# tensorlayer/HyperPose

Hardware: AMD Instinct MI355X
Metric: end-to-end FPS (preproc+DNN+PAF parse) @ 368x432 (higher is better)
Workload: dtype f32; 1 GPU; configs[1]: Lightweight-OpenPose (MobilenetDilated) + PAF parser, batch 8 @ 368x432 per GPU; frames from pinned host memory (one H2D per batch), parser on the network's own maps, humans to the host; key=configs[1]/f32, global_batch=8, parallelism=frame-sharded x1, no steady-state collective, pipes_per_gpu=4, parser_input=the network's own heat-maps

## Files before the change

hyperpose_amd/csrc/conv32_epilogue.hpp:

```cpp
#pragma once
#include "conv_fp32.hpp"

#include "conv_device.hpp"

namespace hp {

typedef float f32x4e __attribute__((ext_vector_type(4)));

template <int TM>
struct rows_geom {
    static constexpr int CH = TM * 32, PITCH = CH + 4, LPR = CH / 4, RPP = 64 / LPR, NP = 32 / RPP;
    static constexpr int SLAB_BYTES = 32 * PITCH * 4;
};

template <int TM, int NROWS, class F>
__device__ __forceinline__ void conv32_drain_rows(const conv32_params& p, const float* slab, int lane, int m_base, F&& pixel)
{
    using R = rows_geom<TM>;
    const int c4 = lane % R::LPR, r0 = lane / R::LPR;
    const int m = m_base + c4 * 4;
    const bool any = m < p.Cout, full = m + 3 < p.Cout;
    const bool out_vec = ((p.out.coff | p.out.cs) & 3) == 0, res_vec = p.res.p && ((p.res.coff | p.res.cs) & 3) == 0;
    const f32x4e bs = *reinterpret_cast<const f32x4e*>(p.bias + m);
    f32x4e sl = { p.act_slope, p.act_slope, p.act_slope, p.act_slope };
    if (p.alpha)
        sl = *reinterpret_cast<const f32x4e*>(p.alpha + m);
    constexpr int NPASS = NROWS / R::RPP, GRP = NPASS < 4 ? NPASS : NPASS % 4 == 0 ? 4 : NPASS % 3 == 0 ? 3 : 1;
    static_assert(NROWS % R::RPP == 0 && NPASS % GRP == 0, "slab rows per pass");
#pragma unroll
    for (int g = 0; g < NPASS; g += GRP) {
        f32x4e v[GRP], rr[GRP];
        bool ok[GRP];
        long ooff[GRP];
#pragma unroll
        for (int k = 0; k < GRP; ++k) {
            const int r = (g + k) * R::RPP + r0;
            long roff = 0;
            pixel(r, ok[k], ooff[k], roff);
            ok[k] = ok[k] && any;
            v[k] = *reinterpret_cast<const f32x4e*>(slab + r * R::PITCH + c4 * 4);
            rr[k] = f32x4e{ 0.f, 0.f, 0.f, 0.f };
            if (p.res.p && ok[k]) {
                if (full && res_vec)
                    rr[k] = *reinterpret_cast<const f32x4e*>(p.res.p + roff + m);
                else {
#pragma unroll
                    for (int e = 0; e < 4; ++e)
                        if (m + e < p.Cout)
                            rr[k][e] = p.res.p[roff + m + e];
                }
            }
        }
#pragma unroll
        for (int k = 0; k < GRP; ++k) {
            f32x4e o;
#pragma unroll
            for (int e = 0; e < 4; ++e) {
                float x = v[k][e] + bs[e];
                if (p.res.p && p.res_before_act)
                    x += rr[k][e];
                x = x > 0.f ? fminf(x, p.act_hi) : x * sl[e];
                if (p.res.p && !p.res_before_act)
                    x += rr[k][e];
                o[e] = x;
            }
            if (ok[k]) {
                if (full && out_vec)
                    *reinterpret_cast<f32x4e*>(p.out.p + ooff[k] + m) = o;
                else {
#pragma unroll
                    for (int e = 0; e < 4; ++e)
                        if (m + e < p.Cout)
                            p.out.p[ooff[k] + m + e] = o[e];
                }
            }
        }
    }
}

template <int TM, class F>
__device__ __forceinline__ void conv32_store_rows(const conv32_params& p, const floatx16 (&acc)[TM], float* slab, int lane, int m_base, F&& pixel)
{
    using R = rows_geom<TM>;
    const int n = lane & 31, fk = lane >> 5;
#pragma unroll
    for (int i = 0; i < TM; ++i)
#pragma unroll
        for (int q = 0; q < 4; ++q)
            *reinterpret_cast<f32x4e*>(slab + n * R::PITCH + 32 * i + 8 * q + 4 * fk) = f32x4e{ acc[i][4 * q], acc[i][4 * q + 1], acc[i][4 * q + 2], acc[i][4 * q + 3] };
    asm volatile("s_waitcnt lgkmcnt(0)" ::: "memory");
    conv32_drain_rows<TM, 32>(p, slab, lane, m_base, pixel);
}

}
```

hyperpose_amd/csrc/conv_fp32.hip:

```cpp
#include "conv_fp32.hpp"

#include "conv32_epilogue.hpp"
#include "conv_device.hpp"

#include <algorithm>
#include <cstdlib>

namespace hp {

namespace {

typedef float f32x4 __attribute__((ext_vector_type(4)));

__device__ __forceinline__ float act32(float v, int act, float param, float alpha)
{
    switch (act) {
    case ACT_RELU:
        return fmaxf(v, 0.f);
    case ACT_RELU6:
        return fminf(fmaxf(v, 0.f), 6.f);
    case ACT_LEAKY:
        return v > 0.f ? v : v * param;
    case ACT_PRELU:
        return v > 0.f ? v : v * alpha;
    case ACT_SIGMOID:
        return 1.f / (1.f + expf(-v));
    case ACT_SOFTPLUS:
        return v > 20.f ? v : log1pf(expf(v));
    default:
        return v;
    }
}

__device__ __forceinline__ long tv32_off(const tview32& t, int b, int y, int x)
{
    return ((long)b * t.img + (long)y * t.wp + x) * t.cs + t.coff;
}

}

template <int BM, int BN, int WM, int WN, bool ROWS>
__global__ __launch_bounds__(256) void conv32_kernel(const conv32_params p)
{
    constexpr int BK = 16, LDR = 20;
    constexpr int TM = BM / WM / 32, TN = BN / WN / 32, NA = BM / 64, NB = BN / 64;
    static_assert(WM * WN == 4 && TM >= 1 && TN >= 1 && NA >= 1 && NB >= 1, "tile");
    constexpr int AB_BYTES = 2 * (BM + BN) * LDR * 4, SLABS = 4 * rows_geom<TM>::SLAB_BYTES;
    __shared__ __attribute__((aligned(16))) unsigned char lds_raw[AB_BYTES > SLABS ? AB_BYTES : SLABS];
    float (*const sA)[BM * LDR] = reinterpret_cast<float (*)[BM * LDR]>(lds_raw);
    float (*const sB)[BN * LDR] = reinterpret_cast<float (*)[BN * LDR]>(lds_raw + 2 * BM * LDR * 4);

    const int tid = threadIdx.x, lane = tid & 63, wave = tid >> 6;
    const int wm = wave / WN, wn = wave % WN;
    const int G = p.Cout_pad / BM, nx = (p.npix + BN - 1) / BN;
    const int bj = blockIdx.x >> 3, ptile = (bj / G) * 8 + (blockIdx.x & 7);
    if (ptile >= nx)
        return;
    const int n0 = ptile * BN, m0 = (bj % G) * BM;
    const int lrow = tid >> 2, lchunk = (tid & 3) * 4;
    const int OHW = p.OH * p.OW, kc = p.Cin / BK, steps = p.KH * p.KW * kc;

    long bbase[NB];
#pragma unroll
    for (int j = 0; j < NB; ++j) {
        const int n = min(n0 + lrow + 64 * j, p.npix - 1);
        const int b = n / OHW, rem = n - b * OHW;
        const int oy = rem / p.OW, ox = rem - oy * p.OW;
        bbase[j] = tv32_off(p.in, b, oy * p.stride - p.pad_t, ox * p.stride - p.pad_l) + lchunk;
    }
    const float* const wrow = p.w + (long)(m0 + lrow) * p.Cin + lchunk;

    f32x4 ra[NA], rb[NB];
    auto gload = [&](int s) {
        const int tap = s / kc, k0 = (s - tap * kc) * BK;
        const int ky = tap / p.KW, kx = tap - ky * p.KW;
        const long toff = ((long)(ky * p.dil) * p.in.wp + kx * p.dil) * p.in.cs + k0;
        const float* const wt = wrow + (long)tap * p.Cout_pad * p.Cin + k0;
#pragma unroll
        for (int j = 0; j < NA; ++j)
            ra[j] = *reinterpret_cast<const f32x4*>(wt + (long)(64 * j) * p.Cin);
#pragma unroll
        for (int j = 0; j < NB; ++j)
            rb[j] = *reinterpret_cast<const f32x4*>(p.in.p + bbase[j] + toff);
    };
    auto to_lds = [&](int buf) {
#pragma unroll
        for (int j = 0; j < NA; ++j)
            *reinterpret_cast<f32x4*>(&sA[buf][(lrow + 64 * j) * LDR + lchunk]) = ra[j];
#pragma unroll
        for (int j = 0; j < NB; ++j)
            *reinterpret_cast<f32x4*>(&sB[buf][(lrow + 64 * j) * LDR + lchunk]) = rb[j];
    };

    floatx16 acc[TM][TN];
#pragma unroll
    for (int i = 0; i < TM; ++i)
#pragma unroll
        for (int j = 0; j < TN; ++j)
#pragma unroll
            for (int r = 0; r < 16; ++r)
                acc[i][j][r] = 0.f;

    const int frow = lane & 31, fh = (lane >> 5) * 4;
    int dbg_i = 0;
#define HP_STAMP()                                       \
    if (p.dbg && blockIdx.x == 9 && tid == 0)            \
        p.dbg[dbg_i++] = __builtin_amdgcn_s_memtime();
    HP_STAMP();
    if (p.dbg && tid == 0 && blockIdx.x < 4096) {
        p.dbg[128 + 3 * blockIdx.x] = __builtin_amdgcn_s_memrealtime();
        p.dbg[128 + 3 * blockIdx.x + 2] = ((unsigned long long)__builtin_amdgcn_s_getreg((31 << 11) | 20) << 32) | (unsigned)__builtin_amdgcn_s_getreg((31 << 11) | 4);
    }
    gload(0);
    to_lds(0);
    lds_barrier();
    HP_STAMP();
#pragma unroll 1
    for (int s = 0; s < steps; ++s) {
        gload(min(s + 1, steps - 1));
        const float* const a_s = &sA[s & 1][(wm * TM * 32 + frow) * LDR + fh];
        const float* const b_s = &sB[s & 1][(wn * TN * 32 + frow) * LDR + fh];
#pragma unroll
        for (int kk = 0; kk < BK / 8; ++kk) {
            f32x4 fa[TM], fb[TN];
#pragma unroll
            for (int i = 0; i < TM; ++i)
                fa[i] = *reinterpret_cast<const f32x4*>(a_s + i * 32 * LDR + kk * 8);
#pragma unroll
            for (int j = 0; j < TN; ++j)
                fb[j] = *reinterpret_cast<const f32x4*>(b_s + j * 32 * LDR + kk * 8);
#pragma unroll
            for (int e = 0; e < 4; ++e)
#pragma unroll
                for (int i = 0; i < TM; ++i)
#pragma unroll
                    for (int j = 0; j < TN; ++j)
                        acc[i][j] = __builtin_amdgcn_mfma_f32_32x32x2f32(fa[i][e], fb[j][e], acc[i][j], 0, 0, 0);
        }
        to_lds((s + 1) & 1);
        lds_barrier();
        if ((s & 7) == 7)
            HP_STAMP();
    }

    if constexpr (ROWS) {
        lds_barrier();
        float* const slab = reinterpret_cast<float*>(lds_raw) + wave * (rows_geom<TM>::SLAB_BYTES / 4);
#pragma unroll
        for (int j = 0; j < TN; ++j) {
            floatx16 fin[TM];
#pragma unroll
            for (int i = 0; i < TM; ++i)
                fin[i] = acc[i][j];
            const int nb = n0 + (wn * TN + j) * 32;
            conv32_store_rows<TM>(p, fin, slab, lane, m0 + wm * TM * 32, [&](int r, bool& ok, long& ooff, long& roff) {
                const int n = nb + r;
                ok = n < p.npix;
                const int nc = min(n, p.npix - 1);
                const int b = nc / OHW, rem = nc - b * OHW;
                const int oy = rem / p.OW, ox = rem - oy * p.OW;
                ooff = tv32_off(p.out, b, oy, ox);
                roff = p.res.p ? tv32_off(p.res, b, oy, ox) : 0;
            });
        }
    } else {
    const bool out_vec = p.out.p && ((p.out.coff | p.out.cs) & 3) == 0;
    const bool res_vec = p.res.p && ((p.res.coff | p.res.cs) & 3) == 0;
    const bool res_pre = p.res.p && p.res_before_act, res_post = p.res.p && !p.res_before_act;
#pragma unroll
    for (int j = 0; j < TN; ++j) {
        const int n = n0 + (wn * TN + j) * 32 + frow;
        const bool pix_ok = n < p.npix;
        const int nc = min(n, p.npix - 1);
        const int b = nc / OHW, rem = nc - b * OHW;
        const int oy = rem / p.OW, ox = rem - oy * p.OW;
        const long ooff = p.out.p ? tv32_off(p.out, b, oy, ox) : 0;
        const long roff = p.res.p ? tv32_off(p.res, b, oy, ox) : 0;
#pragma unroll
        for (int i = 0; i < TM; ++i) {
#pragma unroll
            for (int q = 0; q < 4; ++q) {
                const int m = m0 + (wm * TM + i) * 32 + 8 * q + fh;
                if (pix_ok && m < p.Cout) {
                    const bool full = m + 3 < p.Cout;
                    float v[4], rr[4] = { 0.f, 0.f, 0.f, 0.f };
                    if (p.res.p) {
                        if (full && res_vec) {
                            const f32x4 t = *reinterpret_cast<const f32x4*>(p.res.p + roff + m);
                            rr[0] = t[0], rr[1] = t[1], rr[2] = t[2], rr[3] = t[3];
                        } else {
#pragma unroll
                            for (int e = 0; e < 4; ++e)
                                if (m + e < p.Cout)
                                    rr[e] = p.res.p[roff + m + e];
                        }
                    }
                    const f32x4 bs = *reinterpret_cast<const f32x4*>(p.bias + m);
                    f32x4 sl = { p.act_slope, p.act_slope, p.act_slope, p.act_slope };
                    if (p.alpha)
                        sl = *reinterpret_cast<const f32x4*>(p.alpha + m);
#pragma unroll
                    for (int e = 0; e < 4; ++e) {
                        float x = acc[i][j][4 * q + e] + bs[e];
                        if (res_pre)
                            x += rr[e];
                        x = x > 0.f ? fminf(x, p.act_hi) : x * sl[e];
                        if (res_post)
                            x += rr[e];
                        v[e] = x;
                    }
                    if (p.out.p) {
                        if (full && out_vec) {
                            f32x4 t = { v[0], v[1], v[2], v[3] };
                            *reinterpret_cast<f32x4*>(p.out.p + ooff + m) = t;
                        } else {
#pragma unroll
                            for (int e = 0; e < 4; ++e)
                                if (m + e < p.Cout)
                                    p.out.p[ooff + m + e] = v[e];
                        }
                    }
                    if (p.out_f32) {
#pragma unroll
                        for (int e = 0; e < 4; ++e)
                            if (m + e < p.Cout)
                                p.out_f32[((long)b * p.Cout + m + e) * OHW + rem] = v[e];
                    }
                }
            }
        }
    }
    }
    HP_STAMP();
    if (p.dbg && tid == 0 && blockIdx.x < 4096)
        p.dbg[128 + 3 * blockIdx.x + 1] = __builtin_amdgcn_s_memrealtime();
#undef HP_STAMP
}

template <int BN, int WN = 2>
__global__ __launch_bounds__(256) void conv32_t16_kernel(const conv32_params p)
{
    constexpr int BM = 64, BK = 16, WM = 4 / WN, TMW = BM / 16 / WM, TNW = BN / WN / 16;
    constexpr int NB = (BN + 63) / 64, BR = NB * 64;
    static_assert(BN % (16 * WN) == 0 && (WN == 1 || WN == 2), "wavefront columns of whole 16-pixel tiles");
    __shared__ __attribute__((aligned(16))) float lds[2 * (BM + BR) * BK];
    float (*const sA)[BM * BK] = reinterpret_cast<float (*)[BM * BK]>(lds);
    float (*const sB)[BR * BK] = reinterpret_cast<float (*)[BR * BK]>(lds + 2 * BM * BK);

    const int tid = threadIdx.x, lane = tid & 63, wave = tid >> 6;
    const int wm = WN == 2 ? wave >> 1 : wave, wn = WN == 2 ? wave & 1 : 0;
    const int G = p.Cout_pad / BM, nx = (p.npix + BN - 1) / BN;
    const int bj = blockIdx.x >> 3, ptile = (bj / G) * 8 + (blockIdx.x & 7);
    if (ptile >= nx)
        return;
    const int n0 = ptile * BN, m0 = (bj % G) * BM;
    const int lrow = tid >> 2, lq = tid & 3;
    const int OHW = p.OH * p.OW, kc = p.Cin / BK, steps = p.KH * p.KW * kc;
    auto swz = [](int row, int quad) { return row * BK + ((quad ^ (((row >> 3) & 1) << 1)) << 2); };

    long bbase[NB];
#pragma unroll
    for (int j = 0; j < NB; ++j) {
        const int n = min(n0 + min(lrow + 64 * j, BN - 1), p.npix - 1);
        const int b = n / OHW, rem = n - b * OHW;
        const int oy = rem / p.OW, ox = rem - oy * p.OW;
        bbase[j] = tv32_off(p.in, b, oy * p.stride - p.pad_t, ox * p.stride - p.pad_l) + lq * 4;
    }
    const float* const wrow = p.w + (long)(m0 + lrow) * p.Cin + lq * 4;
    f32x4 ra, rb[NB];
    auto gload = [&](int s) {
        const int tap = s / kc, k0 = (s - tap * kc) * BK;
        const int ky = tap / p.KW, kx = tap - ky * p.KW;
        const long toff = ((long)(ky * p.dil) * p.in.wp + kx * p.dil) * p.in.cs + k0;
        ra = *reinterpret_cast<const f32x4*>(wrow + (long)tap * p.Cout_pad * p.Cin + k0);
#pragma unroll
        for (int j = 0; j < NB; ++j)
            rb[j] = *reinterpret_cast<const f32x4*>(p.in.p + bbase[j] + toff);
    };
    auto to_lds = [&](int buf) {
        *reinterpret_cast<f32x4*>(&sA[buf][swz(lrow, lq)]) = ra;
#pragma unroll
        for (int j = 0; j < NB; ++j)
            *reinterpret_cast<f32x4*>(&sB[buf][swz(lrow + 64 * j, lq)]) = rb[j];
    };

    f32x4 acc[TMW][TNW];
#pragma unroll
    for (int i = 0; i < TMW; ++i)
#pragma unroll
        for (int j = 0; j < TNW; ++j)
            acc[i][j] = f32x4{ 0.f, 0.f, 0.f, 0.f };

    const int fr = lane & 15, kq = lane >> 4;
    int dbg_i = 0;
#define HP_STAMP()                                       \
    if (p.dbg && blockIdx.x == 9 && tid == 0)            \
        p.dbg[dbg_i++] = __builtin_amdgcn_s_memtime();
    HP_STAMP();
    if (p.dbg && tid == 0 && blockIdx.x < 4096) {
        p.dbg[128 + 3 * blockIdx.x] = __builtin_amdgcn_s_memrealtime();
        p.dbg[128 + 3 * blockIdx.x + 2] = ((unsigned long long)__builtin_amdgcn_s_getreg((31 << 11) | 20) << 32) | (unsigned)__builtin_amdgcn_s_getreg((31 << 11) | 4);
    }
    gload(0);
    to_lds(0);
    lds_barrier();
    HP_STAMP();
#pragma unroll 1
    for (int s = 0; s < steps; ++s) {
        gload(min(s + 1, steps - 1));
        f32x4 fa[TMW], fb[TNW];
#pragma unroll
        for (int i = 0; i < TMW; ++i)
            fa[i] = *reinterpret_cast<const f32x4*>(&sA[s & 1][swz(wm * (16 * TMW) + i * 16 + fr, kq)]);
#pragma unroll
        for (int j = 0; j < TNW; ++j)
            fb[j] = *reinterpret_cast<const f32x4*>(&sB[s & 1][swz(wn * (BN / WN) + j * 16 + fr, kq)]);
#pragma unroll
        for (int e = 0; e < 4; ++e)
#pragma unroll
            for (int i = 0; i < TMW; ++i)
#pragma unroll
                for (int j = 0; j < TNW; ++j)
                    acc[i][j] = __builtin_amdgcn_mfma_f32_16x16x4f32(fa[i][e], fb[j][e], acc[i][j], 0, 0, 0);
        to_lds((s + 1) & 1);
        lds_barrier();
        if ((s & 7) == 7)
            HP_STAMP();
    }

    const int q = lane >> 4;
    const bool out_vec = p.out.p && ((p.out.coff | p.out.cs) & 3) == 0;
    const bool res_vec = p.res.p && ((p.res.coff | p.res.cs) & 3) == 0;
    const bool res_pre = p.res.p && p.res_before_act, res_post = p.res.p && !p.res_before_act;
    f32x4 bs[TMW], sl[TMW];
#pragma unroll
    for (int i = 0; i < TMW; ++i) {
        const int m = m0 + wm * (16 * TMW) + i * 16 + 4 * q;
        bs[i] = *reinterpret_cast<const f32x4*>(p.bias + m);
        sl[i] = f32x4{ p.act_slope, p.act_slope, p.act_slope, p.act_slope };
        if (p.alpha)
            sl[i] = *reinterpret_cast<const f32x4*>(p.alpha + m);
    }
#pragma unroll
    for (int j = 0; j < TNW; ++j) {
        const int n = n0 + wn * (BN / WN) + j * 16 + fr;
        const bool pix_ok = n < p.npix;
        const int nc = min(n, p.npix - 1);
        const int b = nc / OHW, rem = nc - b * OHW;
        const int oy = rem / p.OW, ox = rem - oy * p.OW;
        const long ooff = p.out.p ? tv32_off(p.out, b, oy, ox) : 0;
        const long roff = p.res.p ? tv32_off(p.res, b, oy, ox) : 0;
#pragma unroll
        for (int i = 0; i < TMW; ++i) {
            const int m = m0 + wm * (16 * TMW) + i * 16 + 4 * q;
            if (!pix_ok || m >= p.Cout)
                continue;
            const bool full = m + 3 < p.Cout;
            float v[4], rr[4] = { 0.f, 0.f, 0.f, 0.f };
            if (p.res.p) {
                if (full && res_vec) {
                    const f32x4 t = *reinterpret_cast<const f32x4*>(p.res.p + roff + m);
                    rr[0] = t[0], rr[1] = t[1], rr[2] = t[2], rr[3] = t[3];
                } else {
#pragma unroll
                    for (int e = 0; e < 4; ++e)
                        if (m + e < p.Cout)
                            rr[e] = p.res.p[roff + m + e];
                }
            }
#pragma unroll
            for (int e = 0; e < 4; ++e) {
                float x = acc[i][j][e] + bs[i][e];
                if (res_pre)
                    x += rr[e];
                x = x > 0.f ? fminf(x, p.act_hi) : x * sl[i][e];
                if (res_post)
                    x += rr[e];
                v[e] = x;
            }
            if (p.out.p) {
                if (full && out_vec)
                    *reinterpret_cast<f32x4*>(p.out.p + ooff + m) = f32x4{ v[0], v[1], v[2], v[3] };
                else {
#pragma unroll
                    for (int e = 0; e < 4; ++e)
                        if (m + e < p.Cout)
                            p.out.p[ooff + m + e] = v[e];
                }
            }
            if (p.out_f32) {
#pragma unroll
                for (int e = 0; e < 4; ++e)
                    if (m + e < p.Cout)
                        p.out_f32[((long)b * p.Cout + m + e) * OHW + rem] = v[e];
            }
        }
    }
    HP_STAMP();
    if (p.dbg && tid == 0 && blockIdx.x < 4096)
        p.dbg[128 + 3 * blockIdx.x + 1] = __builtin_amdgcn_s_memrealtime();
#undef HP_STAMP
}

template <int KT, int BN>
__global__ __launch_bounds__(256) void conv32_wk_kernel(const conv32_params p)
{
    constexpr int BM = 64, KS = KT / 16, CPR = KT / 4, TMW = 4, TNW = BN / 64, WPX = BN / 4;
    constexpr int SA = BM * 16 + 16, SB = BN * 16 + 16;
    constexpr int SLAB = 16 * 36;
    constexpr int NA = BM * CPR / 256, NBC = (BN * CPR + 255) / 256;
    static_assert(BN % 64 == 0 && KT % 16 == 0 && (BM * CPR) % 256 == 0, "tile shape");
    extern __shared__ __attribute__((aligned(16))) float lds[];
    float* const sA = lds;
    float* const sB = lds + KS * SA;
    long* const s_in = reinterpret_cast<long*>(lds + KS * (SA + SB) + 4 * SLAB);
    long* const s_out = s_in + BN;
    long* const s_res = s_out + BN;

    const int tid = threadIdx.x, lane = tid & 63, wave = tid >> 6;
    float* const slab = lds + KS * (SA + SB) + wave * SLAB;
    const int G = p.Cout_pad / BM, nx = (p.npix + BN - 1) / BN;
    const int bj = blockIdx.x >> 3, ptile = (bj / G) * 8 + (blockIdx.x & 7);
    if (ptile >= nx)
        return;
    const int n0 = ptile * BN, m0 = (bj % G) * BM;
    const int OHW = p.OH * p.OW;
    auto swz = [](int row, int quad) { return row * 16 + ((quad ^ (((row >> 3) & 1) << 1)) << 2); };

    if (tid < BN) {
        const int n = min(n0 + tid, p.npix - 1);
        const int b = n / OHW, rem = n - b * OHW;
        const int oy = rem / p.OW, ox = rem - oy * p.OW;
        s_in[tid] = tv32_off(p.in, b, oy * p.stride - p.pad_t, ox * p.stride - p.pad_l);
        s_out[tid] = tv32_off(p.out, b, oy, ox);
        s_res[tid] = p.res.p ? tv32_off(p.res, b, oy, ox) : 0;
    }
    const int fr = lane & 15, kq = lane >> 4;
    const int rrow = lane >> 3, rc = lane & 7;
    const bool out_vec = ((p.out.coff | p.out.cs) & 3) == 0;
    const bool res_vec = p.res.p && ((p.res.coff | p.res.cs) & 3) == 0 && p.res.coff + p.Cout_pad <= p.res.cs;
    const bool res_pre = p.res.p && p.res_before_act, res_post = p.res.p && !p.res_before_act;
    f32x4 bsr[2], slr[2];
#pragma unroll
    for (int h = 0; h < 2; ++h) {
        const int m = m0 + h * 32 + 4 * rc;
        bsr[h] = *reinterpret_cast<const f32x4*>(p.bias + m);
        slr[h] = f32x4{ p.act_slope, p.act_slope, p.act_slope, p.act_slope };
        if (p.alpha)
            slr[h] = *reinterpret_cast<const f32x4*>(p.alpha + m);
    }
    f32x4 va[NA], vb[NBC];
#pragma unroll
    for (int i = 0; i < NA; ++i) {
        const int idx = tid + 256 * i, row = idx / CPR, c = idx % CPR;
        va[i] = *reinterpret_cast<const f32x4*>(p.w + (long)(m0 + row) * p.Cin + c * 4);
    }
    __syncthreads();
#pragma unroll
    for (int i = 0; i < NBC; ++i) {
        const int idx = min(tid + 256 * i, BN * CPR - 1), row = idx / CPR, c = idx % CPR;
        vb[i] = *reinterpret_cast<const f32x4*>(p.in.p + s_in[row] + c * 4);
    }
    f32x4 rr[TNW][2][2];
    if (res_vec) {
#pragma unroll
        for (int j = 0; j < TNW; ++j)
#pragma unroll
            for (int r = 0; r < 2; ++r) {
                const long roff = s_res[wave * WPX + j * 16 + 8 * r + rrow] + m0 + 4 * rc;
#pragma unroll
                for (int h = 0; h < 2; ++h)
                    rr[j][h][r] = *reinterpret_cast<const f32x4*>(p.res.p + roff + h * 32);
            }
    }
#pragma unroll
    for (int i = 0; i < NA; ++i) {
        const int idx = tid + 256 * i, row = idx / CPR, c = idx % CPR;
        *reinterpret_cast<f32x4*>(&sA[(c >> 2) * SA + swz(row, c & 3)]) = va[i];
    }
#pragma unroll
    for (int i = 0; i < NBC; ++i) {
        const int idx = tid + 256 * i, row = idx / CPR, c = idx % CPR;
        if (idx < BN * CPR)
            *reinterpret_cast<f32x4*>(&sB[(c >> 2) * SB + swz(row, c & 3)]) = vb[i];
    }
    __syncthreads();

#pragma unroll
    for (int j = 0; j < TNW; ++j) {
        f32x4 acc[TMW];
#pragma unroll
        for (int i = 0; i < TMW; ++i)
            acc[i] = f32x4{ 0.f, 0.f, 0.f, 0.f };
        const int prow0 = wave * WPX + j * 16;
#pragma unroll
        for (int s = 0; s < KS; ++s) {
            f32x4 fa[TMW];
#pragma unroll
            for (int i = 0; i < TMW; ++i)
                fa[i] = *reinterpret_cast<const f32x4*>(&sA[s * SA + swz(i * 16 + fr, kq)]);
            const f32x4 fb = *reinterpret_cast<const f32x4*>(&sB[s * SB + swz(prow0 + fr, kq)]);
#pragma unroll
            for (int e = 0; e < 4; ++e)
#pragma unroll
                for (int i = 0; i < TMW; ++i)
                    acc[i] = __builtin_amdgcn_mfma_f32_16x16x4f32(fa[i][e], fb[e], acc[i], 0, 0, 0);
        }
#pragma unroll
        for (int h = 0; h < 2; ++h) {
#pragma unroll
            for (int i = 0; i < 2; ++i)
                *reinterpret_cast<f32x4*>(&slab[fr * 36 + i * 16 + 4 * kq]) = acc[2 * h + i];
            __builtin_amdgcn_wave_barrier();
#pragma unroll
            for (int r = 0; r < 2; ++r) {
                const f32x4 a = *reinterpret_cast<const f32x4*>(&slab[(8 * r + rrow) * 36 + 4 * rc]);
                const int prow = prow0 + 8 * r + rrow, m = m0 + h * 32 + 4 * rc;
                if (n0 + prow >= p.npix || m >= p.Cout)
                    continue;
                const bool full = m + 3 < p.Cout;
                const long ooff = s_out[prow] + m;
                float v[4], rv[4] = { 0.f, 0.f, 0.f, 0.f };
                if (p.res.p) {
                    if (res_vec) {
                        rv[0] = rr[j][h][r][0], rv[1] = rr[j][h][r][1], rv[2] = rr[j][h][r][2], rv[3] = rr[j][h][r][3];
                    } else {
                        const long roff = s_res[prow] + m;
#pragma unroll
                        for (int e = 0; e < 4; ++e)
                            if (m + e < p.Cout)
                                rv[e] = p.res.p[roff + e];
                    }
                }
#pragma unroll
                for (int e = 0; e < 4; ++e) {
                    float x = a[e] + bsr[h][e];
                    if (res_pre)
                        x += rv[e];
                    x = x > 0.f ? fminf(x, p.act_hi) : x * slr[h][e];
                    if (res_post)
                        x += rv[e];
                    v[e] = x;
                }
                if (full && out_vec)
                    *reinterpret_cast<f32x4*>(p.out.p + ooff) = f32x4{ v[0], v[1], v[2], v[3] };
                else {
#pragma unroll
                    for (int e = 0; e < 4; ++e)
                        if (m + e < p.Cout)
                            p.out.p[ooff + e] = v[e];
                }
            }
            __builtin_amdgcn_wave_barrier();
        }
    }
}

template <int KT, int BN>
static hipError_t launch_wk(const conv32_params& p, dim3 grid, hipStream_t s)
{
    constexpr int lds = KT / 16 * ((64 * 16 + 16) + (BN * 16 + 16)) * 4 + 4 * 16 * 36 * 4 + 3 * BN * 8;
    static bool granted = false;
    if (lds > 64 * 1024 && !granted) {
        const hipError_t e = hipFuncSetAttribute((const void*)conv32_wk_kernel<KT, BN>, hipFuncAttributeMaxDynamicSharedMemorySize, lds);
        if (e != hipSuccess)
            return e;
        granted = true;
    }
    HP_LAUNCH((conv32_wk_kernel<KT, BN>), grid, dim3(256), lds, s, p);
    return hipGetLastError();
}

static int conv32_wk_bn(const conv32_params& p, const engine_switches& sw)
{
    const int wk = sw.c32_wk;
    if (wk == 0 || p.KH != 1 || p.KW != 1 || p.dil != 1 || p.out_f32 || !p.out.p || (p.Cin != 32 && p.Cin != 64 && p.Cin != 128))
        return 0;
    if (p.Cin == 128 && wk != 1)
        return 0;
    const int bn = 64;
    const long np = p.pick_npix > 0 ? p.pick_npix : p.npix, blocks = (np + bn - 1) / bn * (p.Cout_pad / 64);
    return wk == 1 || blocks >= 768 ? bn : 0;
}

static void conv32_pick(const conv32_params& p, const engine_switches& sw, int& BM, int& BN)
{
    BM = p.Cout_pad % 128 == 0 ? 128 : 64, BN = 128;
    const long blocks = (long)(((p.pick_npix > 0 ? p.pick_npix : p.npix) + 127) / 128) * (p.Cout_pad / BM);
    if (blocks < 448)
        BM = 64, BN = 64;
    else if (blocks < 1024 && BM == 128)
        BM = 64;
    const int bn160 = sw.c32_bn160;
    if (bn160 == 1 || bn160 == 176) {
        BM = 64, BN = bn160 == 1 ? 160 : 176;
        return;
    }
    if (BM == 64 && BN == 128 && bn160 != 0) {
        const long np = p.pick_npix > 0 ? p.pick_npix : p.npix;
        const long g = p.Cout_pad / 64, b128 = (long)((np + 127) / 128) * g, b160 = (long)((np + 159) / 160) * g;
        if (b128 > 1024 && b160 <= 1024)
            BN = 160;
    }
    if (bn160 != 0 && p.KH == 1 && p.KW == 1 && p.stride == 1 && p.Cin <= 128 && p.Cout_pad >= 256 && !p.out_f32 && (BN == 128))
        BM = 64, BN = 160;
}

static bool conv32_rows(const conv32_params& p, int BN)
{
    if (BN == 160 || BN == 176)
        return false;
    return !p.out_f32 && (p.lane_epilogue < 0 || (p.lane_epilogue == 0 && BN == 64));
}

int conv32_tile(const conv32_params& p, const engine_switches& sw)
{
    if (const int bn = conv32_wk_bn(p, sw))
        return 39000000 + p.Cin * 1000 + bn;
    int BM, BN;
    conv32_pick(p, sw, BM, BN);
    return 32000000 + (conv32_rows(p, BN) ? 400000 : 0) + BM * 1000 + BN;
}

bool set_act32(conv32_params& p)
{
    const float inf = __builtin_huge_valf();
    switch (p.act) {
    case ACT_NONE:
        p.act_slope = 1.f, p.act_hi = inf;
        return true;
    case ACT_RELU:
        p.act_slope = 0.f, p.act_hi = inf;
        return true;
    case ACT_RELU6:
        p.act_slope = 0.f, p.act_hi = 6.f;
        return true;
    case ACT_LEAKY:
        p.act_slope = p.act_param, p.act_hi = inf;
        return true;
    case ACT_PRELU:
        p.act_slope = 0.f, p.act_hi = inf;
        return p.alpha != nullptr;
    default:
        return false;
    }
}

hipError_t launch_conv32(const conv32_params& p, const engine_switches& sw, hipStream_t s)
{
    if (p.Cin % 16 || p.Cout_pad % 64 || p.npix <= 0)
        return hipErrorInvalidValue;
    if (const int bn = conv32_wk_bn(p, sw)) {
        const dim3 g(((p.npix + bn - 1) / bn + 7) / 8 * 8 * (p.Cout_pad / 64));
        return p.Cin == 32 ? launch_wk<32, 64>(p, g, s) : p.Cin == 64 ? launch_wk<64, 64>(p, g, s) : launch_wk<128, 64>(p, g, s);
    }
    int BM, BN;
    conv32_pick(p, sw, BM, BN);
    const dim3 grid(((p.npix + BN - 1) / BN + 7) / 8 * 8 * (p.Cout_pad / BM));
    const bool rows = conv32_rows(p, BN);
#define HP_C32_CASE(BM_, BN_, WM_, WN_)                                                    \
    if (rows)                                                                              \
        HP_LAUNCH((conv32_kernel<BM_, BN_, WM_, WN_, true>), grid, dim3(256), 0, s, p);    \
    else                                                                                   \
        HP_LAUNCH((conv32_kernel<BM_, BN_, WM_, WN_, false>), grid, dim3(256), 0, s, p);
    if (BN == 176) {
        HP_LAUNCH((conv32_t16_kernel<176, 1>), grid, dim3(256), 0, s, p);
    } else if (BN == 160) {
        HP_LAUNCH((conv32_t16_kernel<160>), grid, dim3(256), 0, s, p);
    } else if (BM == 128) {
        HP_C32_CASE(128, 128, 2, 2)
    } else if (BN == 128) {
        HP_C32_CASE(64, 128, 1, 4)
    } else {
        HP_C32_CASE(64, 64, 2, 2)
    }
#undef HP_C32_CASE
    return hipGetLastError();
}

__device__ unsigned g_first_conv_verify[4];
__global__ __launch_bounds__(256) void first_conv32_kernel(const first_conv32_params p, int tiles_x, int tiles_y, int TH, int GP, int verify)
{
    extern __shared__ __attribute__((aligned(16))) float s_w32[];
    constexpr int TW = 8, PX = 4;
    const int G = (p.Cout + 7) / 8, CP = G * 8, taps = p.KH * p.KW;
    const int IH = (TH - 1) * p.stride + p.KH, IW = (TW - 1) * p.stride + p.KW;
    float* const s_x = s_w32 + taps * 3 * CP;
    int t = blockIdx.x;
    const int tx = t % tiles_x;
    t /= tiles_x;
    const int ty = t % tiles_y, b = t / tiles_y;
    const int oy0 = ty * TH, ox0 = tx * TW;
    const int iy0 = oy0 * p.stride - p.pad_t, ix0 = ox0 * p.stride - p.pad_l;
    for (int i = threadIdx.x; i < taps * 3 * CP; i += 256) {
        const int co = i % CP, tc = i / CP;
        s_w32[i] = co < p.Cout ? p.w[(size_t)co * taps * 3 + tc] : 0.f;
    }
    for (int i = threadIdx.x; i < IH * IW; i += 256) {
// ... 422 lines not shown
```

Measured before the change: 5393 frames/s.

## Restructure conv epilogues: batched residual loads, incremental pixel indexing, global address space

Result: faster. 5476 frames/s, median of 6 (+1.5%).

```diff
diff --git a/hyperpose_amd/csrc/conv32_epilogue.hpp b/hyperpose_amd/csrc/conv32_epilogue.hpp
--- a/hyperpose_amd/csrc/conv32_epilogue.hpp
+++ b/hyperpose_amd/csrc/conv32_epilogue.hpp
@@ -6,6 +6,8 @@
 namespace hp {
 
 typedef float f32x4e __attribute__((ext_vector_type(4)));
+typedef __attribute__((address_space(1))) float gfloat_e;
+typedef __attribute__((address_space(1))) f32x4e gf32x4e;
 
 template <int TM>
 struct rows_geom {
@@ -13,73 +15,113 @@
     static constexpr int SLAB_BYTES = 32 * PITCH * 4;
 };
 
-template <int TM, int NROWS, class F>
-__device__ __forceinline__ void conv32_drain_rows(const conv32_params& p, const float* slab, int lane, int m_base, F&& pixel)
+struct no_stamp {
+    __device__ __forceinline__ void operator()() const {}
+};
+
+template <int TM, int NROWS, class F, class S = no_stamp>
+__device__ __forceinline__ void conv32_drain_rows(const conv32_params& p, const float* slab, int lane, int m_base, F&& pixel, S&& stamp = S{})
 {
     using R = rows_geom<TM>;
     const int c4 = lane % R::LPR, r0 = lane / R::LPR;
     const int m = m_base + c4 * 4;
-    const bool any = m < p.Cout, full = m + 3 < p.Cout;
+    const bool any = m < p.Cout, full = m + 3 < p.Cout, quads = (p.Cout & 3) == 0;
     const bool out_vec = ((p.out.coff | p.out.cs) & 3) == 0, res_vec = p.res.p && ((p.res.coff | p.res.cs) & 3) == 0;
-    const f32x4e bs = *reinterpret_cast<const f32x4e*>(p.bias + m);
+    const bool res_pre = p.res.p && p.res_before_act, res_post = p.res.p && !p.res_before_act;
+    const f32x4e bs = *(const gf32x4e*)(p.bias + m);
     f32x4e sl = { p.act_slope, p.act_slope, p.act_slope, p.act_slope };
     if (p.alpha)
-        sl = *reinterpret_cast<const f32x4e*>(p.alpha + m);
-    constexpr int NPASS = NROWS / R::RPP, GRP = NPASS < 4 ? NPASS : NPASS % 4 == 0 ? 4 : NPASS % 3 == 0 ? 3 : 1;
-    static_assert(NROWS % R::RPP == 0 && NPASS % GRP == 0, "slab rows per pass");
+        sl = *(const gf32x4e*)(p.alpha + m);
+    auto finish = [&](f32x4e v, f32x4e rr) {
+        f32x4e o;
 #pragma unroll
-    for (int g = 0; g < NPASS; g += GRP) {
-        f32x4e v[GRP], rr[GRP];
-        bool ok[GRP];
-        long ooff[GRP];
+        for (int e = 0; e < 4; ++e) {
+            float x = v[e] + bs[e];
+            if (res_pre)
+                x += rr[e];
+            x = x > 0.f ? fminf(x, p.act_hi) : x * sl[e];
+            if (res_post)
+                x += rr[e];
+            o[e] = x;
+        }
+        return o;
+    };
+    constexpr int NPASS = NROWS / R::RPP;
+    static_assert(NROWS % R::RPP == 0, "slab rows per pass");
+    if (quads && out_vec && (!p.res.p || res_vec)) {
+        const gfloat_e* const gres = (const gfloat_e*)p.res.p;
+        gfloat_e* const gout = (gfloat_e*)p.out.p;
+        const int mc = any ? m : 0;
+        constexpr int GRP = NPASS < 4 ? NPASS : NPASS % 4 == 0 ? 4 : NPASS % 3 == 0 ? 3 : 1;
+        static_assert(NPASS % GRP == 0, "passes per group");
 #pragma unroll
-        for (int k = 0; k < GRP; ++k) {
-            const int r = (g + k) * R::RPP + r0;
-            long roff = 0;
-            pixel(r, ok[k], ooff[k], roff);
-            ok[k] = ok[k] && any;
-            v[k] = *reinterpret_cast<const f32x4e*>(slab + r * R::PITCH + c4 * 4);
-            rr[k] = f32x4e{ 0.f, 0.f, 0.f, 0.f };
-            if (p.res.p && ok[k]) {
-                if (full && res_vec)
-                    rr[k] = *reinterpret_cast<const f32x4e*>(p.res.p + roff + m);
-                else {
+        for (int g = 0; g < NPASS; g += GRP) {
+            f32x4e v[GRP], rr[GRP];
+            bool ok[GRP];
+            long ooff[GRP], roff[GRP];
 #pragma unroll
-                    for (int e = 0; e < 4; ++e)
-                        if (m + e < p.Cout)
-                            rr[k][e] = p.res.p[roff + m + e];
-                }
+            for (int k = 0; k < GRP; ++k) {
+                roff[k] = 0;
+                pixel((g + k) * R::RPP + r0, ok[k], ooff[k], roff[k]);
+                ok[k] = ok[k] && any;
+            }
+            stamp();
+#pragma unroll
+            for (int k = 0; k < GRP; ++k) {
+                v[k] = *reinterpret_cast<const f32x4e*>(slab + ((g + k) * R::RPP + r0) * R::PITCH + c4 * 4);
+                rr[k] = f32x4e{ 0.f, 0.f, 0.f, 0.f };
+            }
+            if (gres) {
+#pragma unroll
+                for (int k = 0; k < GRP; ++k)
+                    rr[k] = *reinterpret_cast<const gf32x4e*>(gres + (roff[k] + mc));
+            }
+            stamp();
+#pragma unroll
+            for (int k = 0; k < GRP; ++k)
+                v[k] = finish(v[k], rr[k]);
+            stamp();
+#pragma unroll
+            for (int k = 0; k < GRP; ++k)
+                if (ok[k])
+                    *reinterpret_cast<gf32x4e*>(gout + (ooff[k] + m)) = v[k];
+        }
+        return;
+    }
+#pragma unroll
+    for (int k = 0; k < NPASS; ++k) {
+        const int r = k * R::RPP + r0;
+        bool ok;
+        long ooff, roff = 0;
+        pixel(r, ok, ooff, roff);
+        ok = ok && any;
+        f32x4e rr = { 0.f, 0.f, 0.f, 0.f };
+        if (p.res.p && ok) {
+            if (full && res_vec)
+                rr = *reinterpret_cast<const f32x4e*>(p.res.p + roff + m);
+            else {
+#pragma unroll
+                for (int e = 0; e < 4; ++e)
+                    if (m + e < p.Cout)
+                        rr[e] = p.res.p[roff + m + e];
             }
         }
+        const f32x4e o = finish(*reinterpret_cast<const f32x4e*>(slab + r * R::PITCH + c4 * 4), rr);
+        if (ok) {
+            if (full && out_vec)
+                *reinterpret_cast<f32x4e*>(p.out.p + ooff + m) = o;
+            else {
 #pragma unroll
-        for (int k = 0; k < GRP; ++k) {
-            f32x4e o;
-#pragma unroll
-            for (int e = 0; e < 4; ++e) {
-                float x = v[k][e] + bs[e];
-                if (p.res.p && p.res_before_act)
-                    x += rr[k][e];
-                x = x > 0.f ? fminf(x, p.act_hi) : x * sl[e];
-                if (p.res.p && !p.res_before_act)
-                    x += rr[k][e];
-                o[e] = x;
-            }
-            if (ok[k]) {
-                if (full && out_vec)
-                    *reinterpret_cast<f32x4e*>(p.out.p + ooff[k] + m) = o;
-                else {
-#pragma unroll
-                    for (int e = 0; e < 4; ++e)
-                        if (m + e < p.Cout)
-                            p.out.p[ooff[k] + m + e] = o[e];
-                }
+                for (int e = 0; e < 4; ++e)
+                    if (m + e < p.Cout)
+                        p.out.p[ooff + m + e] = o[e];
             }
         }
     }
 }
 
-template <int TM, class F>
-__device__ __forceinline__ void conv32_store_rows(const conv32_params& p, const floatx16 (&acc)[TM], float* slab, int lane, int m_base, F&& pixel)
+template <int TM, class F, class S = no_stamp>
+__device__ __forceinline__ void conv32_store_rows(const conv32_params& p, const floatx16 (&acc)[TM], float* slab, int lane, int m_base, F&& pixel, S&& stamp = S{})
 {
     using R = rows_geom<TM>;
     const int n = lane & 31, fk = lane >> 5;
@@ -89,7 +131,7 @@
         for (int q = 0; q < 4; ++q)
             *reinterpret_cast<f32x4e*>(slab + n * R::PITCH + 32 * i + 8 * q + 4 * fk) = f32x4e{ acc[i][4 * q], acc[i][4 * q + 1], acc[i][4 * q + 2], acc[i][4 * q + 3] };
     asm volatile("s_waitcnt lgkmcnt(0)" ::: "memory");
-    conv32_drain_rows<TM, 32>(p, slab, lane, m_base, pixel);
+    conv32_drain_rows<TM, 32>(p, slab, lane, m_base, pixel, stamp);
 }
 
 }
diff --git a/hyperpose_amd/csrc/conv_fp32.hip b/hyperpose_amd/csrc/conv_fp32.hip
--- a/hyperpose_amd/csrc/conv_fp32.hip
+++ b/hyperpose_amd/csrc/conv_fp32.hip
@@ -5,12 +5,15 @@
 
 #include <algorithm>
 #include <cstdlib>
+#include <type_traits>
 
 namespace hp {
 
 namespace {
 
 typedef float f32x4 __attribute__((ext_vector_type(4)));
+typedef __attribute__((address_space(1))) float gfloat;
+typedef __attribute__((address_space(1))) f32x4 gf32x4;
 
 __device__ __forceinline__ float act32(float v, int act, float param, float alpha)
 {
@@ -60,6 +63,11 @@
     const int lrow = tid >> 2, lchunk = (tid & 3) * 4;
     const int OHW = p.OH * p.OW, kc = p.Cin / BK, steps = p.KH * p.KW * kc;
 
+    int dbg_i = 0;
+#define HP_STAMP()                                       \
+    if (p.dbg && blockIdx.x == 9 && tid == 0)            \
+        p.dbg[dbg_i++] = __builtin_amdgcn_s_memtime();
+    HP_STAMP();
     long bbase[NB];
 #pragma unroll
     for (int j = 0; j < NB; ++j) {
@@ -102,11 +110,6 @@
                 acc[i][j][r] = 0.f;
 
     const int frow = lane & 31, fh = (lane >> 5) * 4;
-    int dbg_i = 0;
-#define HP_STAMP()                                       \
-    if (p.dbg && blockIdx.x == 9 && tid == 0)            \
-        p.dbg[dbg_i++] = __builtin_amdgcn_s_memtime();
-    HP_STAMP();
     if (p.dbg && tid == 0 && blockIdx.x < 4096) {
         p.dbg[128 + 3 * blockIdx.x] = __builtin_amdgcn_s_memrealtime();
         p.dbg[128 + 3 * blockIdx.x + 2] = ((unsigned long long)__builtin_amdgcn_s_getreg((31 << 11) | 20) << 32) | (unsigned)__builtin_amdgcn_s_getreg((31 << 11) | 4);
@@ -146,6 +149,8 @@
     if constexpr (ROWS) {
         lds_barrier();
         float* const slab = reinterpret_cast<float*>(lds_raw) + wave * (rows_geom<TM>::SLAB_BYTES / 4);
+        int pn = min(n0 + wn * TN * 32 + lane / rows_geom<TM>::LPR, p.npix - 1), pb = pn / OHW;
+        int poy = (pn - pb * OHW) / p.OW, pox = pn - pb * OHW - poy * p.OW;
 #pragma unroll
         for (int j = 0; j < TN; ++j) {
             floatx16 fin[TM];
@@ -154,14 +159,17 @@
                 fin[i] = acc[i][j];
             const int nb = n0 + (wn * TN + j) * 32;
             conv32_store_rows<TM>(p, fin, slab, lane, m0 + wm * TM * 32, [&](int r, bool& ok, long& ooff, long& roff) {
-                const int n = nb + r;
+                const int n = nb + r, nc = min(n, p.npix - 1);
                 ok = n < p.npix;
-                const int nc = min(n, p.npix - 1);
-                const int b = nc / OHW, rem = nc - b * OHW;
-                const int oy = rem / p.OW, ox = rem - oy * p.OW;
-                ooff = tv32_off(p.out, b, oy, ox);
-                roff = p.res.p ? tv32_off(p.res, b, oy, ox) : 0;
-            });
+                pox += nc - pn, pn = nc;
+                while (pox >= p.OW) {
+                    pox -= p.OW;
+                    if (++poy == p.OH)
+                        poy = 0, ++pb;
+                }
+                ooff = tv32_off(p.out, pb, poy, pox);
+                roff = p.res.p ? tv32_off(p.res, pb, poy, pox) : 0;
+            }, [&]() { HP_STAMP(); });
         }
     } else {
     const bool out_vec = p.out.p && ((p.out.coff | p.out.cs) & 3) == 0;
@@ -238,7 +246,7 @@
 }
 
 template <int BN, int WN = 2>
-__global__ __launch_bounds__(256) void conv32_t16_kernel(const conv32_params p)
+__global__ __launch_bounds__(256) __attribute__((amdgpu_waves_per_eu(4, 4))) void conv32_t16_kernel(const conv32_params p)
 {
     constexpr int BM = 64, BK = 16, WM = 4 / WN, TMW = BM / 16 / WM, TNW = BN / WN / 16;
     constexpr int NB = (BN + 63) / 64, BR = NB * 64;
@@ -258,6 +266,11 @@
     const int OHW = p.OH * p.OW, kc = p.Cin / BK, steps = p.KH * p.KW * kc;
     auto swz = [](int row, int quad) { return row * BK + ((quad ^ (((row >> 3) & 1) << 1)) << 2); };
 
+    int dbg_i = 0;
+#define HP_STAMP()                                       \
+    if (p.dbg && blockIdx.x == 9 && tid == 0)            \
+        p.dbg[dbg_i++] = __builtin_amdgcn_s_memtime();
+    HP_STAMP();
     long bbase[NB];
 #pragma unroll
     for (int j = 0; j < NB; ++j) {
@@ -292,11 +305,6 @@
             acc[i][j] = f32x4{ 0.f, 0.f, 0.f, 0.f };
 
     const int fr = lane & 15, kq = lane >> 4;
-    int dbg_i = 0;
-#define HP_STAMP()                                       \
-    if (p.dbg && blockIdx.x == 9 && tid == 0)            \
-        p.dbg[dbg_i++] = __builtin_amdgcn_s_memtime();
-    HP_STAMP();
     if (p.dbg && tid == 0 && blockIdx.x < 4096) {
         p.dbg[128 + 3 * blockIdx.x] = __builtin_amdgcn_s_memrealtime();
         p.dbg[128 + 3 * blockIdx.x + 2] = ((unsigned long long)__builtin_amdgcn_s_getreg((31 << 11) | 20) << 32) | (unsigned)__builtin_amdgcn_s_getreg((31 << 11) | 4);
@@ -329,71 +337,126 @@
     }
 
     const int q = lane >> 4;
-    const bool out_vec = p.out.p && ((p.out.coff | p.out.cs) & 3) == 0;
-    const bool res_vec = p.res.p && ((p.res.coff | p.res.cs) & 3) == 0;
+    const bool quads = (p.Cout & 3) == 0;
+    const bool out_vec = quads && ((p.out.coff | p.out.cs) & 3) == 0, res_vec = quads && ((p.res.coff | p.res.cs) & 3) == 0;
     const bool res_pre = p.res.p && p.res_before_act, res_post = p.res.p && !p.res_before_act;
+    const gfloat* const gres = (const gfloat*)p.res.p;
+    gfloat* const gout = (gfloat*)p.out.p;
+    int opix[TNW], rpix[TNW];
+    bool pok[TNW];
+    {
+        const int n = n0 + wn * (BN / WN) + fr, nc = min(n, p.npix - 1);
+        int b = nc / OHW;
+        const int rem = nc - b * OHW;
+        int oy = rem / p.OW, ox = rem - oy * p.OW;
+        pok[0] = n < p.npix;
+        opix[0] = b * p.out.img + oy * p.out.wp + ox;
+        rpix[0] = b * p.res.img + oy * p.res.wp + ox;
+#pragma unroll
+        for (int j = 1; j < TNW; ++j) {
+            pok[j] = n + 16 * j < p.npix;
+            ox += 16;
+            while (ox >= p.OW) {
+                ox -= p.OW;
+                if (++oy == p.OH)
+                    oy = 0, ++b;
+            }
+            opix[j] = pok[j] ? b * p.out.img + oy * p.out.wp + ox : opix[j - 1];
+            rpix[j] = pok[j] ? b * p.res.img + oy * p.res.wp + ox : rpix[j - 1];
+        }
+    }
+    int mch[TMW];
+    bool many[TMW];
+#pragma unroll
+    for (int i = 0; i < TMW; ++i)
+        mch[i] = m0 + wm * (16 * TMW) + i * 16 + 4 * q, many[i] = mch[i] < p.Cout;
     f32x4 bs[TMW], sl[TMW];
-#pragma unroll
-    for (int i = 0; i < TMW; ++i) {
-        const int m = m0 + wm * (16 * TMW) + i * 16 + 4 * q;
-        bs[i] = *reinterpret_cast<const f32x4*>(p.bias + m);
-        sl[i] = f32x4{ p.act_slope, p.act_slope, p.act_slope, p.act_slope };
-        if (p.alpha)
-            sl[i] = *reinterpret_cast<const f32x4*>(p.alpha + m);
-    }
-#pragma unroll
-    for (int j = 0; j < TNW; ++j) {
-        const int n = n0 + wn * (BN / WN) + j * 16 + fr;
-        const bool pix_ok = n < p.npix;
-        const int nc = min(n, p.npix - 1);
-        const int b = nc / OHW, rem = nc - b * OHW;
-        const int oy = rem / p.OW, ox = rem - oy * p.OW;
-        const long ooff = p.out.p ? tv32_off(p.out, b, oy, ox) : 0;
-        const long roff = p.res.p ? tv32_off(p.res, b, oy, ox) : 0;
-#pragma unroll
-        for (int i = 0; i < TMW; ++i) {
-            const int m = m0 + wm * (16 * TMW) + i * 16 + 4 * q;
-            if (!pix_ok || m >= p.Cout)
-                continue;
-            const bool full = m + 3 < p.Cout;
-            float v[4], rr[4] = { 0.f, 0.f, 0.f, 0.f };
-            if (p.res.p) {
-                if (full && res_vec) {
-                    const f32x4 t = *reinterpret_cast<const f32x4*>(p.res.p + roff + m);
-                    rr[0] = t[0], rr[1] = t[1], rr[2] = t[2], rr[3] = t[3];
-                } else {
-#pragma unroll
-                    for (int e = 0; e < 4; ++e)
-                        if (m + e < p.Cout)
-                            rr[e] = p.res.p[roff + m + e];
+    constexpr int GJ = TMW * TNW <= 10 ? TNW : (TNW + 1) / 2;
+    auto drain = [&](auto J0c, auto J1c) {
+        constexpr int J0 = decltype(J0c)::value, J1 = decltype(J1c)::value;
+        HP_STAMP();
+        f32x4 rr[TMW][GJ];
+#pragma unroll
+        for (int i = 0; i < TMW; ++i)
+#pragma unroll
+            for (int j = J0; j < J1; ++j)
+                rr[i][j - J0] = f32x4{ 0.f, 0.f, 0.f, 0.f };
+        if (gres) {
+            if (res_vec) {
+#pragma unroll
+                for (int j = J0; j < J1; ++j)
+#pragma unroll
+                    for (int i = 0; i < TMW; ++i)
+                        rr[i][j - J0] = *reinterpret_cast<const gf32x4*>(gres + ((long)rpix[j] * p.res.cs + p.res.coff + (many[i] ? mch[i] : 0)));
+            } else {
+#pragma unroll
+                for (int j = J0; j < J1; ++j)
+#pragma unroll
+                    for (int i = 0; i < TMW; ++i)
+#pragma unroll
+                        for (int e = 0; e < 4; ++e)
+                            rr[i][j - J0][e] = gres[(long)rpix[j] * p.res.cs + p.res.coff + min(mch[i] + e, p.Cout - 1)];
+            }
+        }
+        if constexpr (J0 == 0) {
+#pragma unroll
+            for (int i = 0; i < TMW; ++i) {
+                bs[i] = *(const gf32x4*)(p.bias + mch[i]);
+                sl[i] = f32x4{ p.act_slope, p.act_slope, p.act_slope, p.act_slope };
+                if (p.alpha)
+                    sl[i] = *(const gf32x4*)(p.alpha + mch[i]);
+            }
+        }
+        HP_STAMP();
+#pragma unroll
+        for (int i = 0; i < TMW; ++i)
+#pragma unroll
+            for (int j = J0; j < J1; ++j)
+#pragma unroll
+                for (int e = 0; e < 4; ++e) {
+                    float x = acc[i][j][e] + bs[i][e];
+                    if (res_pre)
+                        x += rr[i][j - J0][e];
+                    x = x > 0.f ? fminf(x, p.act_hi) : x * sl[i][e];
+                    if (res_post)
+                        x += rr[i][j - J0][e];
+                    acc[i][j][e] = x;
                 }
-            }
-#pragma unroll
-            for (int e = 0; e < 4; ++e) {
-                float x = acc[i][j][e] + bs[i][e];
-                if (res_pre)
-                    x += rr[e];
-                x = x > 0.f ? fminf(x, p.act_hi) : x * sl[i][e];
-                if (res_post)
-                    x += rr[e];
-                v[e] = x;
-            }
-            if (p.out.p) {
-                if (full && out_vec)
-                    *reinterpret_cast<f32x4*>(p.out.p + ooff + m) = f32x4{ v[0], v[1], v[2], v[3] };
-                else {
-#pragma unroll
-                    for (int e = 0; e < 4; ++e)
-                        if (m + e < p.Cout)
-                            p.out.p[ooff + m + e] = v[e];
-                }
-            }
-            if (p.out_f32) {
+        HP_STAMP();
+        if (gout) {
+            if (out_vec) {
+#pragma unroll
+                for (int j = J0; j < J1; ++j)
+#pragma unroll
+                    for (int i = 0; i < TMW; ++i)
+                        if (pok[j] && many[i])
+                            *reinterpret_cast<gf32x4*>(gout + ((long)opix[j] * p.out.cs + p.out.coff + mch[i])) = acc[i][j];
+            } else {
+#pragma unroll
+                for (int j = J0; j < J1; ++j)
+#pragma unroll
+                    for (int i = 0; i < TMW; ++i)
+#pragma unroll
+                        for (int e = 0; e < 4; ++e)
+                            if (pok[j] && mch[i] + e < p.Cout)
+                                gout[(long)opix[j] * p.out.cs + p.out.coff + mch[i] + e] = acc[i][j][e];
+            }
+        }
+    };
+    drain(std::integral_constant<int, 0>{}, std::integral_constant<int, GJ>{});
+    if constexpr (GJ < TNW)
+        drain(std::integral_constant<int, GJ>{}, std::integral_constant<int, TNW>{});
+    if (p.out_f32) {
+#pragma unroll
+        for (int j = 0; j < TNW; ++j) {
+            const int n = n0 + wn * (BN / WN) + j * 16 + fr, nc = min(n, p.npix - 1);
+            const int b = nc / OHW, rem = nc - b * OHW;
+#pragma unroll
+            for (int i = 0; i < TMW; ++i)
 #pragma unroll
                 for (int e = 0; e < 4; ++e)
-                    if (m + e < p.Cout)
-                        p.out_f32[((long)b * p.Cout + m + e) * OHW + rem] = v[e];
-            }
+                    if (pok[j] && mch[i] + e < p.Cout)
+                        p.out_f32[((long)b * p.Cout + mch[i] + e) * OHW + rem] = acc[i][j][e];
         }
     }
     HP_STAMP();
```
